# GBATZOLIS/conditional_score_diffusion

Hardware: AMD Instinct MI355X
Metric: images/sec for 1000-step PC sampling, ddpm_paired_SR3 score net of celebA_SR3_160 (BASELINE configs[1]), 160x160 (higher is better)
Workload: dtype f16x3 (every operand carried as hi + lo fp16 = 22 significand bits, 3 MFMAs per product, f32 accumulate; f32-class: the per-op test tolerance is the f32 kernel's, network error 1.9e-6 vs the reference); 1 GPU; BASELINE configs[1]: celebA_SR3_160 (ddpm_paired_SR3, nf=96, ch_mult (1,1,2,2,3,3), attn 20/10/5), 1000-step PC (reverse_diffusion + langevin, snr 0.15), batch 64 per GPU, random-init weights, synthetic LR inputs; images_per_gpu=64, global_batch=64, noise=on-device Philox4x32-10, precision_mode=fp16x3

## Files before the change

### conditional_score_diffusion_amd/csrc/attention.hip

```cpp
#include "common.h"

namespace csd {

typedef float floatx16 __attribute__((ext_vector_type(16)));

#define ATT_THREADS 256
#define ATT_KT 32

template <int NCT>
__global__ __launch_bounds__(ATT_THREADS) void attention_kernel(const float* __restrict__ qkv, int ld,
                                                                float* __restrict__ out, int L,
                                                                float scale) {
  constexpr int C = NCT * 32;
  constexpr int KS = C + 4;
  extern __shared__ __attribute__((aligned(16))) float smem[];
  float* const Ks = smem;
  float* const Vs = smem + ATT_KT * KS;

  const int tid = threadIdx.x;
  const int lane = tid & 63;
  const int wave = tid >> 6;
  const int half = lane >> 5;
  const int b = blockIdx.y;
  const int q0 = blockIdx.x * 128 + wave * 32;
  const bool wave_active = q0 < L;
  const int qrow = min(q0 + (lane & 31), L - 1);
  const float* qptr = qkv + ((size_t)b * L + qrow) * ld + half * 4;
  const float* kvbase = qkv + (size_t)b * L * ld;

  floatx16 o[NCT];
#pragma unroll
  for (int n = 0; n < NCT; ++n)
#pragma unroll
    for (int r = 0; r < 16; ++r) o[n][r] = 0.f;
  float m_run = -INFINITY;
  float l_run = 0.f;

  const int ntiles = (L + ATT_KT - 1) / ATT_KT;
  for (int t = 0; t < ntiles; ++t) {
    const int key0 = t * ATT_KT;
    __syncthreads();
    for (int e = tid; e < 2 * ATT_KT * (C / 4); e += ATT_THREADS) {
      const int which = e / (ATT_KT * (C / 4));
      const int r = e - which * ATT_KT * (C / 4);
      const int key = r / (C / 4);
      const int c4 = r - key * (C / 4);
      float4 v = make_float4(0.f, 0.f, 0.f, 0.f);
      if (key0 + key < L)
        v = *reinterpret_cast<const float4*>(kvbase + (size_t)(key0 + key) * ld + (1 + which) * C + c4 * 4);
      *reinterpret_cast<float4*>((which ? Vs : Ks) + key * KS + c4 * 4) = v;
    }
    __syncthreads();
    if (!wave_active) continue;

    floatx16 s;
#pragma unroll
    for (int r = 0; r < 16; ++r) s[r] = 0.f;
    const float* krow = Ks + (lane & 31) * KS + half * 4;
#pragma unroll 4
    for (int c0 = 0; c0 < C; c0 += 8) {
      const float4 a4 = *reinterpret_cast<const float4*>(krow + c0);
      const float4 b4 = *reinterpret_cast<const float4*>(qptr + c0);
      s = __builtin_amdgcn_mfma_f32_32x32x2f32(a4.x, b4.x, s, 0, 0, 0);
      s = __builtin_amdgcn_mfma_f32_32x32x2f32(a4.y, b4.y, s, 0, 0, 0);
      s = __builtin_amdgcn_mfma_f32_32x32x2f32(a4.z, b4.z, s, 0, 0, 0);
      s = __builtin_amdgcn_mfma_f32_32x32x2f32(a4.w, b4.w, s, 0, 0, 0);
    }
    float mt = -INFINITY;
#pragma unroll
    for (int r = 0; r < 16; ++r) {
      const int key = key0 + (r & 3) + 8 * (r >> 2) + 4 * half;
      s[r] = (key < L) ? s[r] * scale : -INFINITY;
      mt = fmaxf(mt, s[r]);
    }
    mt = fmaxf(mt, __shfl_xor(mt, 32));
    const float m_new = fmaxf(m_run, mt);
    const float alpha = expf(m_run - m_new);
    float psum = 0.f;
#pragma unroll
    for (int r = 0; r < 16; ++r) {
      s[r] = expf(s[r] - m_new);
      psum += s[r];
    }
    l_run = l_run * alpha + psum;
    m_run = m_new;
#pragma unroll
    for (int r = 0; r < 16; ++r) {
      const int row = (r & 3) + 8 * (r >> 2) + 4 * half;
      const float ar = __shfl(alpha, row);
#pragma unroll
      for (int n = 0; n < NCT; ++n) o[n][r] *= ar;
    }
#pragma unroll
    for (int r = 0; r < 16; ++r) {
      const float* vrow = Vs + ((r & 3) + 8 * (r >> 2) + 4 * half) * KS + (lane & 31);
#pragma unroll
      for (int n = 0; n < NCT; ++n)
        o[n] = __builtin_amdgcn_mfma_f32_32x32x2f32(s[r], vrow[n * 32], o[n], 0, 0, 0);
    }
  }

  if (!wave_active) return;
  const float l_tot = l_run + __shfl_xor(l_run, 32);
#pragma unroll
  for (int r = 0; r < 16; ++r) {
    const int row = (r & 3) + 8 * (r >> 2) + 4 * half;
    const float lr = __shfl(l_tot, row);
    const int q = q0 + row;
    if (q < L) {
      float* dst = out + ((size_t)b * L + q) * C + (lane & 31);
#pragma unroll
      for (int n = 0; n < NCT; ++n) dst[n * 32] = o[n][r] / lr;
    }
  }
}

template <int NCT>
static int launch_att(const float* qkv, int ld, float* out, int B, int L, hipStream_t s) {
  constexpr int C = NCT * 32;
  const size_t lds = (size_t)2 * ATT_KT * (C + 4) * sizeof(float);
  auto kern = attention_kernel<NCT>;
  static bool attr_set = false;
  if (!attr_set) {
    CSD_CHECK_HIP(hipFuncSetAttribute(reinterpret_cast<const void*>(kern),
                                      hipFuncAttributeMaxDynamicSharedMemorySize, 160 * 1024));
    attr_set = true;
  }
  const float scale = 1.0f / sqrtf((float)C);
  (void)scale;
  const float ref_scale = (float)pow((double)C, -0.5);
  hipLaunchKernelGGL(kern, dim3(cdiv(L, 128), B), dim3(ATT_THREADS), lds, s, qkv, ld, out, L, ref_scale);
  CSD_LAUNCH_CHECK();
  return CSD_OK;
}

typedef _Float16 half8a __attribute__((ext_vector_type(8)));
typedef _Float16 half4a __attribute__((ext_vector_type(4)));

template <int NCT, int NS, int CS>
__global__ __launch_bounds__(ATT_THREADS) void attention16_kernel(const float* __restrict__ qkv, int ld,
                                                                  float* __restrict__ out, int L, float scale) {
  constexpr int C = NCT * 32, KSTEPS = C / 16;
  constexpr int KS = 2 * C + 16;
  constexpr int VS = 80;
  constexpr int KPL = ATT_KT * KS, VPL = C * VS;
  extern __shared__ __attribute__((aligned(16))) char smem16[];
  char* const Kp = smem16;
  char* const Vp = smem16 + NS * KPL;

  const int tid = threadIdx.x;
  const int lane = tid & 63;
  const int wave = tid >> 6;
  const int kb = lane >> 5, l32 = lane & 31;
  const int b = blockIdx.y;
  constexpr int NOT = (NCT + CS - 1) / CS;
  const int n0 = (wave % CS) * NOT;
  const int q0 = blockIdx.x * (128 / CS) + (wave / CS) * 32;
  const bool wave_active = q0 < L;
  const float* kvbase = qkv + (size_t)b * L * ld;

  half8a qh[KSTEPS], ql[NS == 2 ? KSTEPS : 1];
  {
    const float* qptr = kvbase + (size_t)min(q0 + l32, L - 1) * ld + kb * 8;
#pragma unroll
    for (int ks = 0; ks < KSTEPS; ++ks) {
      const float4 a = *reinterpret_cast<const float4*>(qptr + ks * 16);
      const float4 c = *reinterpret_cast<const float4*>(qptr + ks * 16 + 4);
      const float v[8] = {a.x * scale, a.y * scale, a.z * scale, a.w * scale, c.x * scale, c.y * scale, c.z * scale, c.w * scale};
#pragma unroll
      for (int j = 0; j < 8; ++j) {
        const _Float16 h = (_Float16)v[j];
        qh[ks][j] = h;
        if (NS == 2) ql[ks][j] = (_Float16)(v[j] - (float)h);
      }
    }
  }

  floatx16 o[NOT];
#pragma unroll
  for (int n = 0; n < NOT; ++n)
#pragma unroll
    for (int r = 0; r < 16; ++r) o[n][r] = 0.f;
  float m_run = -INFINITY, l_run = 0.f;

  constexpr int NK = NCT;
  constexpr int NVG = (2 * C + ATT_THREADS - 1) / ATT_THREADS;
  float4 prek[NK], prev[NVG][4];
  auto prefetch = [&](int key0) {
#pragma unroll
    for (int i = 0; i < NK; ++i) {
      const int e = tid + i * ATT_THREADS;
      const int key = e / (C / 4), c4 = e - key * (C / 4);
      prek[i] = key0 + key < L ? *reinterpret_cast<const float4*>(kvbase + (size_t)(key0 + key) * ld + C + c4 * 4)
                               : make_float4(0.f, 0.f, 0.f, 0.f);
    }
#pragma unroll
    for (int i = 0; i < NVG; ++i) {
      const int g = tid + i * ATT_THREADS;
      const int m = g & 7, c4 = min(g >> 3, C / 4 - 1);
#pragma unroll
      for (int u = 0; u < 4; ++u) {
        const int key = key0 + 4 * m + u;
        prev[i][u] = key < L ? *reinterpret_cast<const float4*>(kvbase + (size_t)key * ld + 2 * C + c4 * 4)
                             : make_float4(0.f, 0.f, 0.f, 0.f);
      }
    }
  };
  auto commit = [&]() {
#pragma unroll
    for (int i = 0; i < NK; ++i) {
      const int e = tid + i * ATT_THREADS;
      const int key = e / (C / 4), c4 = e - key * (C / 4);
      const float v[4] = {prek[i].x, prek[i].y, prek[i].z, prek[i].w};
      half4a hi, lo;
#pragma unroll
      for (int j = 0; j < 4; ++j) {
        hi[j] = (_Float16)v[j];
        lo[j] = (_Float16)(v[j] - (float)hi[j]);
      }
      *reinterpret_cast<half4a*>(Kp + key * KS + c4 * 8) = hi;
      if (NS == 2) *reinterpret_cast<half4a*>(Kp + KPL + key * KS + c4 * 8) = lo;
    }
#pragma unroll
    for (int i = 0; i < NVG; ++i) {
      const int g = tid + i * ATT_THREADS;
      if (g >= 2 * C) continue;
      const int m = g & 7, c4 = g >> 3;
      const int w = (4 * m) & 15;
      const int pos = ((4 * m) & 16) + 8 * ((w >> 2) & 1) + 4 * (w >> 3);
#pragma unroll
      for (int j = 0; j < 4; ++j) {
        const float v[4] = {j == 0 ? prev[i][0].x : j == 1 ? prev[i][0].y : j == 2 ? prev[i][0].z : prev[i][0].w,
                            j == 0 ? prev[i][1].x : j == 1 ? prev[i][1].y : j == 2 ? prev[i][1].z : prev[i][1].w,
                            j == 0 ? prev[i][2].x : j == 1 ? prev[i][2].y : j == 2 ? prev[i][2].z : prev[i][2].w,
                            j == 0 ? prev[i][3].x : j == 1 ? prev[i][3].y : j == 2 ? prev[i][3].z : prev[i][3].w};
        half4a hi, lo;
#pragma unroll
        for (int u = 0; u < 4; ++u) {
          hi[u] = (_Float16)v[u];
          lo[u] = (_Float16)(v[u] - (float)hi[u]);
        }
        *reinterpret_cast<half4a*>(Vp + (c4 * 4 + j) * VS + pos * 2) = hi;
        if (NS == 2) *reinterpret_cast<half4a*>(Vp + VPL + (c4 * 4 + j) * VS + pos * 2) = lo;
      }
    }
  };

  constexpr bool AHEAD = NCT <= 6;
  const int ntiles = (L + ATT_KT - 1) / ATT_KT;
  if (AHEAD) prefetch(0);
  for (int t = 0; t < ntiles; ++t) {
    const int key0 = t * ATT_KT;
    if (!AHEAD) prefetch(key0);
    __syncthreads();
    commit();
    __syncthreads();
    if (AHEAD && t + 1 < ntiles) prefetch(key0 + ATT_KT);
    if (!wave_active) continue;

    floatx16 s;
#pragma unroll
    for (int r = 0; r < 16; ++r) s[r] = 0.f;
    const char* krow = Kp + l32 * KS + kb * 16;
    half8a ah_n = *reinterpret_cast<const half8a*>(krow), al_n;
    if (NS == 2) al_n = *reinterpret_cast<const half8a*>(krow + KPL);
#pragma unroll
    for (int ks = 0; ks < KSTEPS; ++ks) {
      const half8a ah = ah_n, al = al_n;
      if (ks + 1 < KSTEPS) {
        ah_n = *reinterpret_cast<const half8a*>(krow + (ks + 1) * 32);
        if (NS == 2) al_n = *reinterpret_cast<const half8a*>(krow + KPL + (ks + 1) * 32);
      }
      if (NS == 2) {
        s = __builtin_amdgcn_mfma_f32_32x32x16_f16(al, qh[ks], s, 0, 0, 0);
        s = __builtin_amdgcn_mfma_f32_32x32x16_f16(ah, ql[ks], s, 0, 0, 0);
      }
      s = __builtin_amdgcn_mfma_f32_32x32x16_f16(ah, qh[ks], s, 0, 0, 0);
      __builtin_amdgcn_sched_barrier(0);
    }
    float mt = -INFINITY;
#pragma unroll
    for (int r = 0; r < 16; ++r) {
      const int key = key0 + (r & 3) + 8 * (r >> 2) + 4 * kb;
      s[r] = (key < L) ? s[r] : -INFINITY;
      mt = fmaxf(mt, s[r]);
    }
    mt = fmaxf(mt, __shfl_xor(mt, 32));
    const float m_new = fmaxf(m_run, mt);
    const float alpha = __expf(m_run - m_new);
    float psum = 0.f;
    half8a ph[2], pl[NS == 2 ? 2 : 1];
#pragma unroll
    for (int r = 0; r < 16; ++r) {
      const float pv = __expf(s[r] - m_new);
      psum += pv;
      const _Float16 h = (_Float16)pv;
      ph[r >> 3][r & 7] = h;
      if (NS == 2) pl[r >> 3][r & 7] = (_Float16)(pv - (float)h);
    }
    l_run = l_run * alpha + psum;
    m_run = m_new;
    if (!__all(alpha == 1.0f)) {
#pragma unroll
      for (int r = 0; r < 16; ++r) {
        const float ar = __shfl(alpha, (r & 3) + 8 * (r >> 2) + 4 * kb);
#pragma unroll
        for (int n = 0; n < NOT; ++n) o[n][r] *= ar;
      }
    }
#pragma unroll
    for (int tt = 0; tt < 2; ++tt) {
      const char* vrow = Vp + (n0 * 32 + l32) * VS + (16 * tt + 8 * kb) * 2;
      half8a vh_n = *reinterpret_cast<const half8a*>(vrow), vl_n;
      if (NS == 2) vl_n = *reinterpret_cast<const half8a*>(vrow + VPL);
#pragma unroll
      for (int n = 0; n < NOT; ++n) {
        if (CS > 1 && n0 + n >= NCT) break;
        const half8a vh = vh_n, vl = vl_n;
        if (n + 1 < NOT && (CS == 1 || n0 + n + 1 < NCT)) {
          vh_n = *reinterpret_cast<const half8a*>(vrow + (n + 1) * 32 * VS);
          if (NS == 2) vl_n = *reinterpret_cast<const half8a*>(vrow + VPL + (n + 1) * 32 * VS);
        }
        if (NS == 2) {
          o[n] = __builtin_amdgcn_mfma_f32_32x32x16_f16(pl[tt], vh, o[n], 0, 0, 0);
          o[n] = __builtin_amdgcn_mfma_f32_32x32x16_f16(ph[tt], vl, o[n], 0, 0, 0);
        }
        o[n] = __builtin_amdgcn_mfma_f32_32x32x16_f16(ph[tt], vh, o[n], 0, 0, 0);
        __builtin_amdgcn_sched_barrier(0);
      }
    }
  }

  if (!wave_active) return;
  const float l_tot = l_run + __shfl_xor(l_run, 32);
#pragma unroll
  for (int r = 0; r < 16; ++r) {
    const int row = (r & 3) + 8 * (r >> 2) + 4 * kb;
    const float lr = __shfl(l_tot, row);
    const int q = q0 + row;
    if (q < L) {
      float* dst = out + ((size_t)b * L + q) * C + n0 * 32 + l32;
#pragma unroll
      for (int n = 0; n < NOT; ++n)
        if (CS == 1 || n0 + n < NCT) dst[n * 32] = o[n][r] / lr;
    }
  }
}

template <int NCT, int NS>
static int launch_att16(const float* qkv, int ld, float* out, int B, int L, hipStream_t s) {
  constexpr int C = NCT * 32;
  const size_t lds = (size_t)NS * (ATT_KT * (2 * C + 16) + C * 80);
  constexpr int CS = NCT >= 8 ? 2 : 1;
  auto kern = attention16_kernel<NCT, NS, CS>;
  static bool attr_set = false;
  if (!attr_set) {
    CSD_CHECK_HIP(hipFuncSetAttribute(reinterpret_cast<const void*>(kern),
                                      hipFuncAttributeMaxDynamicSharedMemorySize, 160 * 1024));
    attr_set = true;
  }
  const float ref_scale = (float)pow((double)C, -0.5);
  hipLaunchKernelGGL(kern, dim3(cdiv(L, 128 / CS), B), dim3(ATT_THREADS), lds, s, qkv, ld, out, L, ref_scale);
  CSD_LAUNCH_CHECK();
  return CSD_OK;
}

int attention16_launch(const float* qkv, int ld, float* out, int B, int L, int C, int ns, hipStream_t s) {
  CSD_REQUIRE(C % 32 == 0, "attention: C=%d must be a multiple of 32", C);
  CSD_REQUIRE(L >= 1, "attention: empty sequence");
  CSD_REQUIRE(ns == 1 || ns == 2, "attention16: %d operand planes", ns);
#define CSD_ATT16_CASE(N) case N: return ns == 2 ? launch_att16<N, 2>(qkv, ld, out, B, L, s) : launch_att16<N, 1>(qkv, ld, out, B, L, s);
  switch (C / 32) {
    CSD_ATT16_CASE(1) CSD_ATT16_CASE(2) CSD_ATT16_CASE(3) CSD_ATT16_CASE(4) CSD_ATT16_CASE(6) CSD_ATT16_CASE(8) CSD_ATT16_CASE(9)
    default:
      set_error("attention: C=%d not instantiated (supported: 32,64,96,128,192,256,288)", C);
      return CSD_ERR_INVALID;
  }
#undef CSD_ATT16_CASE
}

int attention_launch(const float* qkv, int ld, float* out, int B, int L, int C, hipStream_t s) {
  CSD_REQUIRE(C % 32 == 0, "attention: C=%d must be a multiple of 32", C);
  CSD_REQUIRE(L >= 1, "attention: empty sequence");
  switch (C / 32) {
    case 1: return launch_att<1>(qkv, ld, out, B, L, s);
    case 2: return launch_att<2>(qkv, ld, out, B, L, s);
    case 3: return launch_att<3>(qkv, ld, out, B, L, s);
    case 4: return launch_att<4>(qkv, ld, out, B, L, s);
    case 6: return launch_att<6>(qkv, ld, out, B, L, s);
    case 8: return launch_att<8>(qkv, ld, out, B, L, s);
    case 9: return launch_att<9>(qkv, ld, out, B, L, s);
    default:
      set_error("attention: C=%d not instantiated (supported: 32,64,96,128,192,256,288)", C);
      return CSD_ERR_INVALID;
  }
}

}
```

Measured before the change: 1.613 images/sec.

## Double-buffer attention K/V tiles and interleave staging with MFMAs via transposed LDS reads

Reworks the fp16x3 attention kernel so each K/V tile is staged into a double-buffered LDS region while the current tile is being computed. The global loads and hi/lo conversion stores are sliced across the QK and PV MFMA steps, which removes one __syncthreads per tile and hides load latency. V is now kept row-major and read with ds_read_tr16_b64 transposed loads, and the padded layout is chosen to avoid bank conflicts. In exchange LDS use doubles, register pressure rises from the prefetch buffers, and waves with no queries now have to loop purely to help with staging.

```diff
diff --git a/conditional_score_diffusion_amd/csrc/attention.hip b/conditional_score_diffusion_amd/csrc/attention.hip
--- a/conditional_score_diffusion_amd/csrc/attention.hip
+++ b/conditional_score_diffusion_amd/csrc/attention.hip
@@ -1,4 +1,5 @@
 #include "common.h"
+#include <type_traits>
 
 namespace csd {
 
@@ -137,20 +138,53 @@
 typedef _Float16 half8a __attribute__((ext_vector_type(8)));
 typedef _Float16 half4a __attribute__((ext_vector_type(4)));
 
+template <int NCT, int NS>
+struct Att16Lds {
+  static constexpr int C = NCT * 32;
+  static constexpr int KS = 2 * C + 16;
+  static constexpr int PL = ATT_KT * KS;
+  static constexpr int K_HI = 0, K_LO = PL;
+  static constexpr int V_HI = NS * PL, V_LO = NS * PL + PL;
+  static constexpr int TILE = 2 * NS * PL;
+  static constexpr int BYTES = 2 * TILE;
+  static_assert(KS % 16 == 0, "16-byte K fragments, 8-byte transposed reads and stores");
+  static_assert((KS / 16) % 2 == 1, "K rows an odd number of 16-byte chunks apart: conflict-free ds_read_b128 fragments");
+  static_assert((4 * (KS / 4)) % 64 == 16, "V rows 4 apart sit 16 banks apart (transposed reads, paired store rows)");
+  static_assert(NS != 2 || NCT != 6 || BYTES == 102400, "C = 192: 2 x 51 200 B");
+  static_assert(NS != 2 || NCT != 9 || BYTES == 151552, "C = 288: 2 x 75 776 B");
+  static_assert(BYTES <= 160 * 1024, "LDS of one CU");
+};
+
+template <int I, int N, class F>
+__device__ __forceinline__ void att_static_for(F&& f) {
+  if constexpr (I < N) {
+    f(std::integral_constant<int, I>{});
+    att_static_for<I + 1, N>(f);
+  }
+}
+
+__device__ __forceinline__ half4a att_lds_read_tr16(const char* p) {
+#if defined(__HIP_DEVICE_COMPILE__)
+  typedef __fp16 fp16x4 __attribute__((ext_vector_type(4)));
+  typedef __attribute__((address_space(3))) fp16x4* lds_ptr;
+  const auto v = __builtin_amdgcn_ds_read_tr16_b64_v4f16((lds_ptr)(p));
+  return __builtin_bit_cast(half4a, v);
+#else
+  return half4a{};
+#endif
+}
+
 template <int NCT, int NS, int CS>
 __global__ __launch_bounds__(ATT_THREADS) void attention16_kernel(const float* __restrict__ qkv, int ld,
                                                                   float* __restrict__ out, int L, float scale) {
+  typedef Att16Lds<NCT, NS> M;
   constexpr int C = NCT * 32, KSTEPS = C / 16;
-  constexpr int KS = 2 * C + 16;
-  constexpr int VS = 80;
-  constexpr int KPL = ATT_KT * KS, VPL = C * VS;
+  constexpr int KS = M::KS, PL = M::PL;
   extern __shared__ __attribute__((aligned(16))) char smem16[];
-  char* const Kp = smem16;
-  char* const Vp = smem16 + NS * KPL;
 
   const int tid = threadIdx.x;
   const int lane = tid & 63;
-  const int wave = tid >> 6;
+  const int wave = __builtin_amdgcn_readfirstlane(tid >> 6);
   const int kb = lane >> 5, l32 = lane & 31;
   const int b = blockIdx.y;
   constexpr int NOT = (NCT + CS - 1) / CS;
@@ -183,101 +217,118 @@
     for (int r = 0; r < 16; ++r) o[n][r] = 0.f;
   float m_run = -INFINITY, l_run = 0.f;
 
-  constexpr int NK = NCT;
-  constexpr int NVG = (2 * C + ATT_THREADS - 1) / ATT_THREADS;
-  float4 prek[NK], prev[NVG][4];
-  auto prefetch = [&](int key0) {
-#pragma unroll
-    for (int i = 0; i < NK; ++i) {
-      const int e = tid + i * ATT_THREADS;
-      const int key = e / (C / 4), c4 = e - key * (C / 4);
-      prek[i] = key0 + key < L ? *reinterpret_cast<const float4*>(kvbase + (size_t)(key0 + key) * ld + C + c4 * 4)
-                               : make_float4(0.f, 0.f, 0.f, 0.f);
-    }
-#pragma unroll
-    for (int i = 0; i < NVG; ++i) {
-      const int g = tid + i * ATT_THREADS;
-      const int m = g & 7, c4 = min(g >> 3, C / 4 - 1);
-#pragma unroll
-      for (int u = 0; u < 4; ++u) {
-        const int key = key0 + 4 * m + u;
-        prev[i][u] = key < L ? *reinterpret_cast<const float4*>(kvbase + (size_t)key * ld + 2 * C + c4 * 4)
-                             : make_float4(0.f, 0.f, 0.f, 0.f);
-      }
-    }
+  constexpr int NP = 2 * NCT, NU = 2 * NP;
+  constexpr int NR = NCT <= 6 ? NP : NCT;
+  const int su = tid >> 3, sc8 = tid & 7;
+  const int kkey = ((su & 1) << 2) | ((su >> 1) & 3) | (su & 24);
+  const int vkey = su;
+  const int st_k = M::K_HI + kkey * KS + sc8 * 8;
+  const int st_v = M::V_HI + (4 * (su & 3) + ((su >> 2) & 3) + (su & 16)) * KS + sc8 * 8;
+  const float* const gk0 = kvbase + C + sc8 * 4;
+  const float* const gv0 = kvbase + 2 * C + sc8 * 4;
+  float4 pre[NR];
+  auto krows = [&](int T) { return gk0 + (size_t)min(T * ATT_KT + kkey, L - 1) * ld; };
+  auto vrows = [&](int T) { return gv0 + (size_t)min(T * ATT_KT + vkey, L - 1) * ld; };
+  struct Rows { const float* k; const float* v; };
+  auto rows = [&](int T) { return Rows{krows(T), vrows(T)}; };
+  auto load_piece = [&](auto ic, const Rows& g) {
+    constexpr int i = decltype(ic)::value;
+    pre[i % NR] = *reinterpret_cast<const float4*>(i < NCT ? g.k + i * 32 : g.v + (i - NCT) * 32);
   };
-  auto commit = [&]() {
-#pragma unroll
-    for (int i = 0; i < NK; ++i) {
-      const int e = tid + i * ATT_THREADS;
-      const int key = e / (C / 4), c4 = e - key * (C / 4);
-      const float v[4] = {prek[i].x, prek[i].y, prek[i].z, prek[i].w};
-      half4a hi, lo;
-#pragma unroll
-      for (int j = 0; j < 4; ++j) {
-        hi[j] = (_Float16)v[j];
-        lo[j] = (_Float16)(v[j] - (float)hi[j]);
-      }
-      *reinterpret_cast<half4a*>(Kp + key * KS + c4 * 8) = hi;
-      if (NS == 2) *reinterpret_cast<half4a*>(Kp + KPL + key * KS + c4 * 8) = lo;
-    }
-#pragma unroll
-    for (int i = 0; i < NVG; ++i) {
-      const int g = tid + i * ATT_THREADS;
-      if (g >= 2 * C) continue;
-      const int m = g & 7, c4 = g >> 3;
-      const int w = (4 * m) & 15;
-      const int pos = ((4 * m) & 16) + 8 * ((w >> 2) & 1) + 4 * (w >> 3);
-#pragma unroll
-      for (int j = 0; j < 4; ++j) {
-        const float v[4] = {j == 0 ? prev[i][0].x : j == 1 ? prev[i][0].y : j == 2 ? prev[i][0].z : prev[i][0].w,
-                            j == 0 ? prev[i][1].x : j == 1 ? prev[i][1].y : j == 2 ? prev[i][1].z : prev[i][1].w,
-                            j == 0 ? prev[i][2].x : j == 1 ? prev[i][2].y : j == 2 ? prev[i][2].z : prev[i][2].w,
-                            j == 0 ? prev[i][3].x : j == 1 ? prev[i][3].y : j == 2 ? prev[i][3].z : prev[i][3].w};
-        half4a hi, lo;
-#pragma unroll
-        for (int u = 0; u < 4; ++u) {
-          hi[u] = (_Float16)v[u];
-          lo[u] = (_Float16)(v[u] - (float)hi[u]);
-        }
-        *reinterpret_cast<half4a*>(Vp + (c4 * 4 + j) * VS + pos * 2) = hi;
-        if (NS == 2) *reinterpret_cast<half4a*>(Vp + VPL + (c4 * 4 + j) * VS + pos * 2) = lo;
-      }
+  auto stage_unit = [&](auto uc, char* sb, const Rows& ga, const Rows& gb) {
+    constexpr int U = decltype(uc)::value, i = U >> 1;
+    char* const dst = sb + (i < NCT ? st_k + i * 64 : st_v + (i - NCT) * 64);
+    const float4 x = pre[i % NR];
+    const float v[4] = {x.x, x.y, x.z, x.w};
+    half4a hi, lo;
+#pragma unroll
+    for (int j = 0; j < 4; ++j) {
+      hi[j] = (_Float16)v[j];
+      lo[j] = (_Float16)(v[j] - (float)hi[j]);
+    }
+    if ((U & 1) == 0) {
+      *reinterpret_cast<half4a*>(dst) = hi;
+    } else {
+      if (NS == 2) *reinterpret_cast<half4a*>(dst + PL) = lo;
+      if constexpr (i + NR < NP) load_piece(std::integral_constant<int, i + NR>{}, ga);
+      else load_piece(std::integral_constant<int, i + NR - NP>{}, gb);
     }
   };
-
-  constexpr bool AHEAD = NCT <= 6;
+  constexpr int NSLOT = KSTEPS + 2 * NOT;
+  auto stage_slot = [&](auto sc, char* sb, const Rows& ga, const Rows& gb) {
+    constexpr int s = decltype(sc)::value, u0 = s * NU / NSLOT, u1 = (s + 1) * NU / NSLOT;
+    att_static_for<u0, u1>([&](auto uc) { stage_unit(uc, sb, ga, gb); });
+  };
+
   const int ntiles = (L + ATT_KT - 1) / ATT_KT;
-  if (AHEAD) prefetch(0);
+  {
+    const Rows ga = rows(0), gb = rows(1);
+    att_static_for<0, NR>([&](auto ic) { load_piece(ic, ga); });
+    att_static_for<0, NU>([&](auto uc) { stage_unit(uc, smem16, ga, gb); });
+  }
+
+  const int tr_off = M::V_HI + (4 * ((lane >> 2) & 3) + kb) * KS + 32 * ((lane >> 4) & 1) + 8 * (lane & 3);
+  const int kr_off = M::K_HI + l32 * KS + kb * 16;
+
+  if (!wave_active) {
+    for (int t = 0; t < ntiles; ++t) {
+      __syncthreads();
+      char* const sb = smem16 + ((t + 1) & 1) * M::TILE;
+      const Rows ga = rows(t + 1), gb = rows(t + 2);
+      att_static_for<0, NU>([&](auto uc) { stage_unit(uc, sb, ga, gb); });
+    }
+    return;
+  }
+
   for (int t = 0; t < ntiles; ++t) {
     const int key0 = t * ATT_KT;
-    if (!AHEAD) prefetch(key0);
     __syncthreads();
-    commit();
-    __syncthreads();
-    if (AHEAD && t + 1 < ntiles) prefetch(key0 + ATT_KT);
-    if (!wave_active) continue;
+    const char* const rb = smem16 + (t & 1) * M::TILE;
+    char* const sb = smem16 + ((t + 1) & 1) * M::TILE;
+    const Rows ga = rows(t + 1), gb = rows(t + 2);
 
     floatx16 s;
 #pragma unroll
     for (int r = 0; r < 16; ++r) s[r] = 0.f;
-    const char* krow = Kp + l32 * KS + kb * 16;
-    half8a ah_n = *reinterpret_cast<const half8a*>(krow), al_n;
-    if (NS == 2) al_n = *reinterpret_cast<const half8a*>(krow + KPL);
-#pragma unroll
-    for (int ks = 0; ks < KSTEPS; ++ks) {
-      const half8a ah = ah_n, al = al_n;
-      if (ks + 1 < KSTEPS) {
-        ah_n = *reinterpret_cast<const half8a*>(krow + (ks + 1) * 32);
-        if (NS == 2) al_n = *reinterpret_cast<const half8a*>(krow + KPL + (ks + 1) * 32);
+    const char* const krow = rb + kr_off;
+    half8a ah[3], al[3];
+    auto kfrag = [&](auto kc) {
+      constexpr int ks = decltype(kc)::value;
+      ah[ks % 3] = *reinterpret_cast<const half8a*>(krow + ks * 32);
+      if (NS == 2) al[ks % 3] = *reinterpret_cast<const half8a*>(krow + M::K_LO + ks * 32);
+    };
+    kfrag(std::integral_constant<int, 0>{});
+    if constexpr (KSTEPS > 1) kfrag(std::integral_constant<int, 1>{});
+    __builtin_amdgcn_sched_barrier(0);
+    att_static_for<0, KSTEPS>([&](auto kc) {
+      constexpr int ks = decltype(kc)::value;
+      if constexpr (ks + 2 < KSTEPS) kfrag(std::integral_constant<int, ks + 2>{});
+      if constexpr (NS == 2) {
+        s = __builtin_amdgcn_mfma_f32_32x32x16_f16(al[ks % 3], qh[ks], s, 0, 0, 0);
+        s = __builtin_amdgcn_mfma_f32_32x32x16_f16(ah[ks % 3], ql[ks], s, 0, 0, 0);
       }
-      if (NS == 2) {
-        s = __builtin_amdgcn_mfma_f32_32x32x16_f16(al, qh[ks], s, 0, 0, 0);
-        s = __builtin_amdgcn_mfma_f32_32x32x16_f16(ah, ql[ks], s, 0, 0, 0);
-      }
-      s = __builtin_amdgcn_mfma_f32_32x32x16_f16(ah, qh[ks], s, 0, 0, 0);
+      s = __builtin_amdgcn_mfma_f32_32x32x16_f16(ah[ks % 3], qh[ks], s, 0, 0, 0);
+      stage_slot(kc, sb, ga, gb);
       __builtin_amdgcn_sched_barrier(0);
-    }
+    });
+
+    constexpr int NG = 2 * NOT;
+    const char* const vtr = rb + tr_off;
+    int voff[NOT];
+#pragma unroll
+    for (int n = 0; n < NOT; ++n) voff[n] = min(n0 + n, NCT - 1) * 64;
+    half8a vh[3], vl[3];
+    auto vfrag = [&](auto gc) {
+      constexpr int g = decltype(gc)::value, tt = g / NOT, n = g % NOT;
+      const char* const p = vtr + tt * 16 * KS + voff[n];
+      vh[g % 3] = __builtin_shufflevector(att_lds_read_tr16(p), att_lds_read_tr16(p + 2 * KS), 0, 1, 2, 3, 4, 5, 6, 7);
+      if (NS == 2)
+        vl[g % 3] = __builtin_shufflevector(att_lds_read_tr16(p + PL), att_lds_read_tr16(p + PL + 2 * KS), 0, 1, 2, 3, 4, 5, 6, 7);
+    };
+    vfrag(std::integral_constant<int, 0>{});
+    vfrag(std::integral_constant<int, 1>{});
+    __builtin_amdgcn_sched_barrier(0);
+
     float mt = -INFINITY;
 #pragma unroll
     for (int r = 0; r < 16; ++r) {
@@ -308,30 +359,19 @@
         for (int n = 0; n < NOT; ++n) o[n][r] *= ar;
       }
     }
-#pragma unroll
-    for (int tt = 0; tt < 2; ++tt) {
-      const char* vrow = Vp + (n0 * 32 + l32) * VS + (16 * tt + 8 * kb) * 2;
-      half8a vh_n = *reinterpret_cast<const half8a*>(vrow), vl_n;
-      if (NS == 2) vl_n = *reinterpret_cast<const half8a*>(vrow + VPL);
-#pragma unroll
-      for (int n = 0; n < NOT; ++n) {
-        if (CS > 1 && n0 + n >= NCT) break;
-        const half8a vh = vh_n, vl = vl_n;
-        if (n + 1 < NOT && (CS == 1 || n0 + n + 1 < NCT)) {
-          vh_n = *reinterpret_cast<const half8a*>(vrow + (n + 1) * 32 * VS);
-          if (NS == 2) vl_n = *reinterpret_cast<const half8a*>(vrow + VPL + (n + 1) * 32 * VS);
-        }
-        if (NS == 2) {
-          o[n] = __builtin_amdgcn_mfma_f32_32x32x16_f16(pl[tt], vh, o[n], 0, 0, 0);
-          o[n] = __builtin_amdgcn_mfma_f32_32x32x16_f16(ph[tt], vl, o[n], 0, 0, 0);
-        }
-        o[n] = __builtin_amdgcn_mfma_f32_32x32x16_f16(ph[tt], vh, o[n], 0, 0, 0);
-        __builtin_amdgcn_sched_barrier(0);
+    att_static_for<0, NG>([&](auto gc) {
+      constexpr int g = decltype(gc)::value, tt = g / NOT, n = g % NOT;
+      if constexpr (g + 2 < NG) vfrag(std::integral_constant<int, g + 2>{});
+      if constexpr (NS == 2) {
+        o[n] = __builtin_amdgcn_mfma_f32_32x32x16_f16(pl[tt], vh[g % 3], o[n], 0, 0, 0);
+        o[n] = __builtin_amdgcn_mfma_f32_32x32x16_f16(ph[tt], vl[g % 3], o[n], 0, 0, 0);
       }
-    }
-  }
-
-  if (!wave_active) return;
+      o[n] = __builtin_amdgcn_mfma_f32_32x32x16_f16(ph[tt], vh[g % 3], o[n], 0, 0, 0);
+      stage_slot(std::integral_constant<int, KSTEPS + g>{}, sb, ga, gb);
+      __builtin_amdgcn_sched_barrier(0);
+    });
+  }
+
   const float l_tot = l_run + __shfl_xor(l_run, 32);
 #pragma unroll
   for (int r = 0; r < 16; ++r) {
@@ -350,7 +390,7 @@
 template <int NCT, int NS>
 static int launch_att16(const float* qkv, int ld, float* out, int B, int L, hipStream_t s) {
   constexpr int C = NCT * 32;
-  const size_t lds = (size_t)NS * (ATT_KT * (2 * C + 16) + C * 80);
+  const size_t lds = Att16Lds<NCT, NS>::BYTES;
   constexpr int CS = NCT >= 8 ? 2 : 1;
   auto kern = attention16_kernel<NCT, NS, CS>;
   static bool attr_set = false;
```

After: 1.622 images/sec, median of 6. Within noise of the previous version (+0.5%).
